# lambdaclass/ethrex

Measured on NVIDIA H100. Metric: bn254_g1_msm_points_per_sec, higher is better.
Workload: dtype u32x8 Montgomery (254-bit modular integer)

## Files before the change

ethrex_b200/csrc/msm.cu:

```cuda
#include "common.cuh"
#include "tma.cuh"
#include <cstdlib>

namespace b200zk {

static constexpr int kMaxWindows = 64;
static constexpr uint32_t kMaxPipelineChunks = 64;
static constexpr int kChunk = 16;
static constexpr int kG2MinBlocks = 1;

struct MsmPlan {
  uint32_t c, W, B;
  uint32_t chunk, T;
  uint32_t merged;
  uint32_t Wr;
  uint32_t table_stride;
  uint32_t adaptive;
};

uint32_t precompute_window(size_t n) {
  uint32_t lg = 0;
  while (((size_t)1 << lg) < n) ++lg;
  if (lg >= 20) return 20;
  if (lg <= 6) return 6;
// ... 134 lines not shown
#pragma unroll
    for (int u = 0; u < kScatterIlp; ++u) {
      const size_t t = t0 + u * stride;
      live[u] = t < total_pad;
      code[u] = (live[u] && t < total) ? __ldg(digits + t) : kNoDigit;
      active[u] = code[u] != kNoDigit;
      w[u] = live[u] ? t / n : 0;
      g[u] = (pl.merged ? 0u : (uint32_t)(w[u] * pl.B)) + (code[u] & 0x7fffffffu);
    }
#pragma unroll
    for (int u = 0; u < kScatterIlp; ++u) {
      base[u] = 0; rank[u] = 0; mask[u] = 0;
      if (live[u]) {
        uint32_t cnt = warp_group(g[u], active[u], &rank[u], &mask[u], pl.adaptive != 0);
        if (active[u] && rank[u] == 0) base[u] = atomicAdd(&cursor[g[u]], cnt);
      }
    }
#pragma unroll
    for (int u = 0; u < kScatterIlp; ++u) {
      if (live[u]) {
        uint32_t bs = __shfl_sync(mask[u], base[u], __ffs(mask[u]) - 1);
        const size_t t = t0 + u * stride;
        if (active[u]) idx[bs + rank[u]] = (uint32_t)((t - w[u] * n) + (pl.merged ? w[u] * pl.table_stride : 0)) | (code[u] & 0x80000000u);
      }
    }
  }
}

static constexpr uint32_t kSortTile = 1024;
static constexpr uint32_t kSortMaxW = 16;
static constexpr uint32_t kSortMaxBins = 1024;
static constexpr uint32_t kSortMaxFine = 2048;
static constexpr uint32_t kSortCountSub = 4;
static constexpr int kFineIlp = 8;

struct SortPlan {
  uint32_t fb;
  uint32_t C;
  uint32_t NC;
  uint32_t range;
  uint32_t G;
};
static bool make_sort_plan(size_t n, const MsmPlan& pl, int sm_count, SortPlan* sp) {
  const size_t G = (size_t)pl.Wr * pl.B;
  uint32_t kb = 0;
  while (((size_t)1 << kb) < G) ++kb;
  if (pl.W > kSortMaxW || kb < 12 || n < ((size_t)1 << 16)) return false;
  uint32_t cb = kb > 19 ? 10 : 9;
  if (kb - cb > 11) return false;
  sp->fb = kb - cb;
  sp->C = (uint32_t)((G + ((size_t)1 << sp->fb) - 1) >> sp->fb);
  sp->G = (uint32_t)G;
  uint32_t nc = (uint32_t)sm_count;
  size_t tiles = (n + kSortTile - 1) / kSortTile;
  if (nc > tiles) nc = (uint32_t)tiles;
  size_t per = ((tiles + nc - 1) / nc) * kSortTile;
  sp->NC = (uint32_t)((n + per - 1) / per);
  sp->range = (uint32_t)per;
  return true;
}

B2_D void recode_scalar(const uint32_t s[8], const MsmPlan& pl, uint32_t (&code)[kSortMaxW]) {
  uint32_t carry = 0;
#pragma unroll
  for (uint32_t w = 0; w < kSortMaxW; ++w) {
    code[w] = kNoDigit;
    if (w < pl.W) {
      uint32_t coef = window_bits(s, w, pl.c) + carry;
      carry = 0;
      uint32_t neg = 0, mag = coef;
      if (w + 1 < pl.W && coef >= pl.B) { carry = 1; neg = 0x80000000u; mag = (1u << pl.c) - coef; }
      code[w] = mag ? ((mag - 1) | neg) : kNoDigit;
    }
  }
}

__global__ void __launch_bounds__(kHistTile) msm_sort_count(const void* scalars, size_t n, uint32_t flags, MsmPlan pl, SortPlan sp, uint32_t* cnt) {
  __shared__ __align__(128) uint4 tile[2][kHistTile * 2];
  __shared__ uint64_t bar[2];
  __shared__ uint32_t sh[kSortMaxBins];
  const uint32_t r = blockIdx.x / kSortCountSub, sub = blockIdx.x % kSortCountSub;
  for (uint32_t b = threadIdx.x; b < sp.C; b += kHistTile) sh[b] = 0;
  const size_t lo = (size_t)r * sp.range, hi = lo + sp.range < n ? lo + sp.range : n;
  const size_t tiles_all = lo < hi ? (hi - lo + kHistTile - 1) / kHistTile : 0;
  const size_t per = (tiles_all + kSortCountSub - 1) / kSortCountSub;
  const size_t t0 = sub * per, t1 = t0 + per < tiles_all ? t0 + per : tiles_all;
  if (threadIdx.x == 0) { tma::barrier_init(&bar[0], 1); tma::barrier_init(&bar[1], 1); tma::barrier_init_fence(); }
  __syncthreads();
  auto issue = [&](size_t tl, uint32_t buf) {
    size_t first = lo + tl * kHistTile;
    uint32_t bytes = (uint32_t)((hi - first < kHistTile ? hi - first : kHistTile) * 32);
    tma::barrier_expect(&bar[buf], bytes);
    tma::bulk_load(tile[buf], reinterpret_cast<const uint8_t*>(scalars) + first * 32, bytes, &bar[buf]);
  };
  if (threadIdx.x == 0 && t0 < t1) issue(t0, 0);
  uint32_t it = 0;
  for (size_t tl = t0; tl < t1; ++tl, ++it) {
    const uint32_t buf = it & 1;
    if (threadIdx.x == 0 && tl + 1 < t1) issue(tl + 1, buf ^ 1);
    tma::barrier_wait(&bar[buf], (it >> 1) & 1);
    const size_t i = lo + tl * kHistTile + threadIdx.x;
    if (i < hi) {
      uint32_t s[8], code[kSortMaxW];
      decode_scalar(tile[buf][2 * threadIdx.x], tile[buf][2 * threadIdx.x + 1], flags, s);
      recode_scalar(s, pl, code);
#pragma unroll
      for (uint32_t w = 0; w < kSortMaxW; ++w)
        if (code[w] != kNoDigit) {
          const uint32_t g = (pl.merged ? 0u : w * pl.B) + (code[w] & 0x7fffffffu);
          atomicAdd(&sh[g >> sp.fb], 1u);
        }
    }
    __syncthreads();
  }
  __syncthreads();
  for (uint32_t b = threadIdx.x; b < sp.C; b += kHistTile) if (sh[b]) atomicAdd(&cnt[(size_t)b * sp.NC + r], sh[b]);
}

struct SortCoarseSmem {
  uint2 ent[kSortTile * kSortMaxW];
  uint32_t dst[kSortTile * kSortMaxW];
  uint32_t run_base[kSortMaxBins], tile_cnt[kSortMaxBins], tile_start[kSortMaxBins];
  uint32_t warp_tot[kSortTile / 32];
  uint32_t total;
};
__global__ void __launch_bounds__(kSortTile, 1) msm_sort_coarse(const void* __restrict__ scalars, size_t n, uint32_t flags, MsmPlan pl, SortPlan sp, const uint32_t* __restrict__ base,
                                                               uint2* __restrict__ ent1) {
  extern __shared__ __align__(16) uint8_t smem_raw[];
  SortCoarseSmem& sm = *reinterpret_cast<SortCoarseSmem*>(smem_raw);
  const uint32_t r = blockIdx.x, tid = threadIdx.x;
  const size_t lo = (size_t)r * sp.range, hi = lo + sp.range < n ? lo + sp.range : n;
  const uint32_t fmask = (1u << sp.fb) - 1u;
  for (uint32_t b = tid; b < sp.C; b += kSortTile) { sm.run_base[b] = __ldg(base + (size_t)b * sp.NC + r); sm.tile_cnt[b] = 0; }
  __syncthreads();
  const uint4* sc = reinterpret_cast<const uint4*>(scalars);
  for (size_t t0 = lo; t0 < hi; t0 += kSortTile) {
    const size_t i = t0 + tid;
    uint32_t code[kSortMaxW], rank[kSortMaxW];
    const bool live = i < hi;
#pragma unroll
    for (uint32_t w = 0; w < kSortMaxW; ++w) { code[w] = kNoDigit; rank[w] = 0; }
    if (live) {
      uint32_t s[8];
      decode_scalar(__ldg(sc + 2 * i), __ldg(sc + 2 * i + 1), flags, s);
      recode_scalar(s, pl, code);
#pragma unroll
      for (uint32_t w = 0; w < kSortMaxW; ++w)
        if (code[w] != kNoDigit) {
          const uint32_t g = (pl.merged ? 0u : w * pl.B) + (code[w] & 0x7fffffffu);
          rank[w] = atomicAdd(&sm.tile_cnt[g >> sp.fb], 1u);
        }
    }
    __syncthreads();
    {
      const uint32_t v = tid < sp.C ? sm.tile_cnt[tid] : 0;
      uint32_t incl = v;
#pragma unroll
      for (int o = 1; o < 32; o <<= 1) { uint32_t t = __shfl_up_sync(0xffffffffu, incl, o); if ((tid & 31) >= (unsigned)o) incl += t; }
      if ((tid & 31) == 31) sm.warp_tot[tid >> 5] = incl;
      __syncthreads();
      uint32_t wb = 0;
      for (uint32_t k = 0; k < (tid >> 5); ++k) wb += sm.warp_tot[k];
      if (tid < sp.C) sm.tile_start[tid] = wb + incl - v;
      if (tid == kSortTile - 1) sm.total = wb + incl;
    }
    __syncthreads();
    if (live) {
#pragma unroll
      for (uint32_t w = 0; w < kSortMaxW; ++w)
        if (code[w] != kNoDigit) {
          const uint32_t g = (pl.merged ? 0u : w * pl.B) + (code[w] & 0x7fffffffu);
          const uint32_t b = g >> sp.fb, pos = sm.tile_start[b] + rank[w];
          sm.ent[pos] = make_uint2((uint32_t)(i + (pl.merged ? (size_t)w * pl.table_stride : 0)) | (code[w] & 0x80000000u), g & fmask);
          sm.dst[pos] = sm.run_base[b] + rank[w];
        }
    }
    __syncthreads();
    const uint32_t total = sm.total;
    for (uint32_t t = tid; t < total; t += kSortTile) ent1[sm.dst[t]] = sm.ent[t];
    __syncthreads();
    if (tid < sp.C) { sm.run_base[tid] += sm.tile_cnt[tid]; sm.tile_cnt[tid] = 0; }
    __syncthreads();
  }
}

static constexpr uint32_t kFineTile = 8192;
static constexpr uint32_t kFineSeg = 4 * kFineTile;
struct SortFineSmem {
  uint32_t val[kFineTile], dst[kFineTile];
  uint32_t cur[kSortMaxFine], tcnt[kSortMaxFine], tstart[kSortMaxFine];
  uint32_t warp_tot[32];
  uint32_t total;
};
B2_D void scan_fine_keys(const uint32_t* in, uint32_t* out, uint32_t F, uint32_t* warp_tot, uint32_t* total) {
  const uint32_t tid = threadIdx.x, k0 = 2 * tid, k1 = 2 * tid + 1;
  const uint32_t v0 = k0 < F ? in[k0] : 0, v1 = k1 < F ? in[k1] : 0;
  uint32_t incl = v0 + v1;
#pragma unroll
  for (int o = 1; o < 32; o <<= 1) { uint32_t t = __shfl_up_sync(0xffffffffu, incl, o); if ((tid & 31) >= (unsigned)o) incl += t; }
  if ((tid & 31) == 31) warp_tot[tid >> 5] = incl;
  __syncthreads();
  uint32_t wb = 0;
  for (uint32_t k = 0; k < (tid >> 5); ++k) wb += warp_tot[k];
  const uint32_t ex = wb + incl - v0 - v1;
  if (k0 < F) out[k0] = ex;
  if (k1 < F) out[k1] = ex + v0;
  if (tid == 1023) *total = wb + incl;
  __syncthreads();
}
__global__ void __launch_bounds__(1024) msm_sort_items(const uint32_t* __restrict__ base, SortPlan sp, uint32_t* __restrict__ item_start) {
  __shared__ uint32_t wt[32];
  const uint32_t tid = threadIdx.x;
  uint32_t v = 0;
  if (tid < sp.C) { const uint32_t sz = __ldg(base + (size_t)(tid + 1) * sp.NC) - __ldg(base + (size_t)tid * sp.NC); v = (sz + kFineSeg - 1) / kFineSeg; }
  uint32_t incl = v;
#pragma unroll
  for (int o = 1; o < 32; o <<= 1) { uint32_t t = __shfl_up_sync(0xffffffffu, incl, o); if ((tid & 31) >= (unsigned)o) incl += t; }
  if ((tid & 31) == 31) wt[tid >> 5] = incl;
  __syncthreads();
  uint32_t wb = 0;
  for (uint32_t k = 0; k < (tid >> 5); ++k) wb += wt[k];
  if (tid < sp.C) item_start[tid] = wb + incl - v;
  if (tid == sp.C - 1) item_start[sp.C] = wb + incl;
}
B2_D uint32_t item_bin(const uint32_t* __restrict__ item_start, uint32_t C, uint32_t i) {
  uint32_t lo = 0, hi = C;
  while (hi - lo > 1) { uint32_t mid = (lo + hi) >> 1; if (__ldg(item_start + mid) <= i) lo = mid; else hi = mid; }
  return lo;
}
__global__ void __launch_bounds__(1024, 2) msm_sort_fine_count(const uint2* __restrict__ ent1, SortPlan sp, const uint32_t* __restrict__ base, const uint32_t* __restrict__ item_start,
                                                               uint32_t* __restrict__ cnt2) {
  __shared__ uint32_t fh[kSortMaxFine];
  const uint32_t i = blockIdx.x, tid = threadIdx.x, F = 1u << sp.fb;
  if (i >= __ldg(item_start + sp.C)) return;
  const uint32_t b = item_bin(item_start, sp.C, i);
  const uint32_t bs = __ldg(base + (size_t)b * sp.NC), be = __ldg(base + (size_t)(b + 1) * sp.NC);
  const uint32_t s0 = bs + (i - __ldg(item_start + b)) * kFineSeg, s1 = (be - s0 > kFineSeg) ? s0 + kFineSeg : be;
  for (uint32_t k = tid; k < F; k += 1024) fh[k] = 0;
  __syncthreads();
  for (uint32_t e0 = s0 + tid; e0 < s1; e0 += 1024 * kFineIlp) {
    uint32_t kk[kFineIlp];
#pragma unroll
    for (int u = 0; u < kFineIlp; ++u) { const uint32_t e = e0 + u * 1024; kk[u] = e < s1 ? __ldg(&ent1[e].y) : 0xffffffffu; }
#pragma unroll
    for (int u = 0; u < kFineIlp; ++u) if (kk[u] != 0xffffffffu) atomicAdd(&fh[kk[u]], 1u);
  }
  __syncthreads();
  for (uint32_t k = tid; k < F; k += 1024) cnt2[(size_t)i * F + k] = fh[k];
}
__global__ void __launch_bounds__(256) msm_sort_fine_prefix(SortPlan sp, const uint32_t* __restrict__ item_start, uint32_t* __restrict__ cnt2, uint32_t* __restrict__ hist) {
  const uint32_t F = 1u << sp.fb;
  const size_t t = blockIdx.x * (size_t)blockDim.x + threadIdx.x;
  if (t >= (size_t)sp.C * F) return;
  const uint32_t b = (uint32_t)(t >> sp.fb), k = (uint32_t)t & (F - 1);
  const uint32_t i0 = __ldg(item_start + b), i1 = __ldg(item_start + b + 1);
  uint32_t run = 0;
  for (uint32_t i = i0; i < i1; ++i) {
    const size_t at = (size_t)i * F + k;
    const uint32_t c = cnt2[at];
    cnt2[at] = run;
    run += c;
  }
  if (t < sp.G) hist[t] = run;
}
__global__ void __launch_bounds__(1024, 1) msm_sort_fine_place(const uint2* __restrict__ ent1, SortPlan sp, const uint32_t* __restrict__ base, const uint32_t* __restrict__ item_start,
                                                               const uint32_t* __restrict__ cnt2, const uint32_t* __restrict__ offsets, uint32_t* __restrict__ idx) {
  extern __shared__ __align__(16) uint8_t smem_raw[];
  SortFineSmem& sm = *reinterpret_cast<SortFineSmem*>(smem_raw);
  const uint32_t i = blockIdx.x, tid = threadIdx.x, F = 1u << sp.fb;
  if (i >= __ldg(item_start + sp.C)) return;
  const uint32_t b = item_bin(item_start, sp.C, i);
  const uint32_t bs = __ldg(base + (size_t)b * sp.NC), be = __ldg(base + (size_t)(b + 1) * sp.NC);
  const uint32_t s0 = bs + (i - __ldg(item_start + b)) * kFineSeg, s1 = (be - s0 > kFineSeg) ? s0 + kFineSeg : be;
  for (uint32_t k = tid; k < F; k += 1024) {
    const size_t g = (size_t)b * F + k;
    sm.cur[k] = (g < sp.G ? __ldg(offsets + g) : 0u) + __ldg(cnt2 + (size_t)i * F + k);
    sm.tcnt[k] = 0;
  }
  __syncthreads();
  for (uint32_t t0 = s0; t0 < s1; t0 += kFineTile) {
    uint2 ev[kFineTile / 1024];
    uint32_t rank[kFineTile / 1024];
#pragma unroll
    for (int u = 0; u < (int)(kFineTile / 1024); ++u) {
      const uint32_t e = t0 + u * 1024 + tid;
      ev[u] = e < s1 ? __ldg(ent1 + e) : make_uint2(0u, 0xffffffffu);
    }
#pragma unroll
    for (int u = 0; u < (int)(kFineTile / 1024); ++u) rank[u] = ev[u].y != 0xffffffffu ? atomicAdd(&sm.tcnt[ev[u].y], 1u) : 0u;
    __syncthreads();
    scan_fine_keys(sm.tcnt, sm.tstart, F, sm.warp_tot, &sm.total);
#pragma unroll
    for (int u = 0; u < (int)(kFineTile / 1024); ++u)
      if (ev[u].y != 0xffffffffu) {
        const uint32_t pos = sm.tstart[ev[u].y] + rank[u];
        sm.val[pos] = ev[u].x;
        sm.dst[pos] = sm.cur[ev[u].y] + rank[u];
      }
    __syncthreads();
    const uint32_t total = sm.total;
    for (uint32_t t = tid; t < total; t += 1024) idx[sm.dst[t]] = sm.val[t];
    __syncthreads();
    for (uint32_t k = tid; k < F; k += 1024) { sm.cur[k] += sm.tcnt[k]; sm.tcnt[k] = 0; }
    __syncthreads();
  }
}

static constexpr int kScanThreads = 256, kScanItems = 8, kScanTile = kScanThreads * kScanItems;

B2_D uint32_t scan_value(const uint32_t* in, const uint32_t* aux, size_t i, uint32_t seg, uint32_t shift) {
  uint32_t v = in[i];
  if (!seg) return (v + (1u << shift) - 1u) >> shift;
  return (v != 0 && (aux[i] % seg) != 0) ? 1u : 0u;
}

__global__ void __launch_bounds__(kScanThreads) scan_tile_sums(const uint32_t* in, const uint32_t* aux, size_t G, uint32_t seg, uint32_t shift, uint32_t* tile_sums) {
  __shared__ uint32_t red[kScanThreads / 32];
  size_t base = (size_t)blockIdx.x * kScanTile + (size_t)threadIdx.x * kScanItems;
  uint32_t s = 0;
#pragma unroll
  for (int k = 0; k < kScanItems; ++k) if (base + k < G) s += scan_value(in, aux, base + k, seg, shift);
#pragma unroll
  for (int o = 16; o; o >>= 1) s += __shfl_xor_sync(0xffffffffu, s, o);
  if ((threadIdx.x & 31) == 0) red[threadIdx.x >> 5] = s;
  __syncthreads();
  if (threadIdx.x == 0) {
    uint32_t t = 0;
    for (int k = 0; k < kScanThreads / 32; ++k) t += red[k];
    tile_sums[blockIdx.x] = t;
  }
// ... 684 lines not shown
  B2_LAUNCH(ctx, groth16_assemble_zk, 3, 32, 0, st, (const uint8_t*)d_partials, count, d_g1_terms, d_g2_terms, zk, (uint8_t*)d_out);
  return B200ZK_OK;
}

static inline void phase_mark(b200zk_ctx* ctx, int k, cudaStream_t st) {
  if (ctx->profiling) cudaEventRecord(ctx->ev[k], st);
}

static int g2_pair_knob() {
  static int k = -1;
  if (k < 0) { const char* e = getenv("B200ZK_G2_PAIR"); k = (e && (*e == '0' || *e == '3' || *e == '4')) ? (*e - '0') : 3; }
  return k;
}
template <class F> static size_t resident_slices(const b200zk_ctx* ctx) {
  if (IsFq2<F>::value) { const int k = g2_pair_knob(); return (size_t)ctx->sm_count * (k ? 64u * (unsigned)k : 256u); }
  return (size_t)ctx->sm_count * (sizeof(F) > 32 ? 256u : 512u);
}
template <class F>
static int launch_accumulate(b200zk_ctx* ctx, cudaStream_t st, const void* pts, const uint32_t* idx, const uint32_t* offsets, const uint32_t* run_off, uint32_t G, uint32_t L,
                             size_t slices, void* partials, uint32_t* run_bucket) {
  const unsigned agrid = (unsigned)((slices + 127) / 128);
  if constexpr (IsFq2<F>::value) {
    const int k = g2_pair_knob();
    const unsigned pgrid = (unsigned)((2 * slices + 127) / 128);
    if (k == 3) B2_LAUNCH(ctx, msm_accumulate_g2_pair<3>, pgrid, 128, 0, st, pts, idx, offsets, run_off, G, L, partials, run_bucket);
    else if (k == 4) B2_LAUNCH(ctx, msm_accumulate_g2_pair<4>, pgrid, 128, 0, st, pts, idx, offsets, run_off, G, L, partials, run_bucket);
    else B2_LAUNCH(ctx, (msm_accumulate<F, false, 1>), agrid, 128, 0, st, pts, idx, offsets, run_off, G, L, partials, run_bucket);
  } else {
    B2_LAUNCH(ctx, (msm_accumulate<F, false>), agrid, 128, 0, st, pts, idx, offsets, run_off, G, L, partials, run_bucket);
  }
  return B200ZK_OK;
}

static int legacy_sort_knob() {
  static int knob = -1;
  if (knob < 0) { const char* e = getenv("B200ZK_SORT"); knob = (e && !strcmp(e, "legacy")) ? 1 : 0; }
  return knob;
}
static double chunk_ratio_knob(double dflt) {
  const char* e = getenv("B200ZK_CHUNK_RATIO");
  double r = (e && *e) ? atof(e) : dflt;
  return (r >= 1.0 && r <= 64.0) ? r : dflt;
}
static size_t sort_ctab_bytes(int sm_count) { return (2 * ((size_t)kSortMaxBins * (size_t)sm_count + 1) + kSortMaxBins + 1) * 4; }
static size_t sort_cnt2_bytes(size_t M_max) { return (M_max / kFineSeg + kSortMaxBins + 1) * (size_t)kSortMaxFine * 4; }
static int run_two_level_sort(b200zk_ctx* ctx, const void* d_scalars, size_t n, uint32_t flags, const MsmPlan& pl, const SortPlan& sp, uint32_t* hist, uint32_t* offsets,
                              uint32_t* tsum, uint2* ent1, uint32_t* ctab, uint32_t* cnt2, uint32_t* idx, cudaStream_t st, bool mark) {
  const size_t Gc = (size_t)sp.C * sp.NC, tilesC = (Gc + kScanTile - 1) / kScanTile;
  const size_t G = sp.G, tilesG = (G + kScanTile - 1) / kScanTile;
  uint32_t *cnt = ctab, *base = ctab + Gc + 1, *item_start = base + Gc + 1;
  if (!ctx->attr_sort) {
    B2_CUDA(ctx, cudaFuncSetAttribute(msm_sort_coarse, cudaFuncAttributeMaxDynamicSharedMemorySize, (int)sizeof(SortCoarseSmem)));
    B2_CUDA(ctx, cudaFuncSetAttribute(msm_sort_fine_place, cudaFuncAttributeMaxDynamicSharedMemorySize, (int)sizeof(SortFineSmem)));
    ctx->attr_sort = true;
  }
  B2_CUDA(ctx, cudaMemsetAsync(cnt, 0, (Gc + 1) * 4, st));
  B2_LAUNCH(ctx, msm_sort_count, sp.NC * kSortCountSub, kHistTile, 0, st, d_scalars, n, flags, pl, sp, cnt);
  if (mark) phase_mark(ctx, 1, st);
  B2_LAUNCH(ctx, scan_tile_sums, (unsigned)tilesC, kScanThreads, 0, st, (const uint32_t*)cnt, (const uint32_t*)nullptr, Gc, 0u, 0u, tsum);
  B2_LAUNCH(ctx, scan_tile_offsets, 1, 1024, 0, st, tsum, tilesC);
  B2_LAUNCH(ctx, scan_apply, (unsigned)tilesC, kScanThreads, 0, st, (const uint32_t*)cnt, (const uint32_t*)nullptr, Gc, 0u, 0u, (const uint32_t*)tsum, base, (uint32_t*)nullptr);
  if (mark) phase_mark(ctx, 2, st);
  B2_LAUNCH(ctx, msm_sort_coarse, sp.NC, kSortTile, sizeof(SortCoarseSmem), st, d_scalars, n, flags, pl, sp, (const uint32_t*)base, ent1);
  const unsigned max_items = (unsigned)((n * (size_t)pl.W) / kFineSeg + sp.C + 1);
  const uint32_t F = 1u << sp.fb;
  B2_LAUNCH(ctx, msm_sort_items, 1, 1024, 0, st, (const uint32_t*)base, sp, item_start);
  B2_LAUNCH(ctx, msm_sort_fine_count, max_items, 1024, 0, st, (const uint2*)ent1, sp, (const uint32_t*)base, (const uint32_t*)item_start, cnt2);
  B2_LAUNCH(ctx, msm_sort_fine_prefix, (unsigned)(((size_t)sp.C * F + 255) / 256), 256, 0, st, sp, (const uint32_t*)item_start, cnt2, hist);
  B2_LAUNCH(ctx, scan_tile_sums, (unsigned)tilesG, kScanThreads, 0, st, (const uint32_t*)hist, (const uint32_t*)nullptr, G, 0u, 0u, tsum);
  B2_LAUNCH(ctx, scan_tile_offsets, 1, 1024, 0, st, tsum, tilesG);
  B2_LAUNCH(ctx, scan_apply, (unsigned)tilesG, kScanThreads, 0, st, (const uint32_t*)hist, (const uint32_t*)nullptr, G, 0u, 0u, (const uint32_t*)tsum, offsets, (uint32_t*)nullptr);
  B2_LAUNCH(ctx, msm_sort_fine_place, max_items, 1024, sizeof(SortFineSmem), st, (const uint2*)ent1, sp, (const uint32_t*)base, (const uint32_t*)item_start, (const uint32_t*)cnt2,
            (const uint32_t*)offsets, idx);
  return B200ZK_OK;
}

template <class F>
static int msm_run_pipelined(b200zk_ctx* ctx, const void* d_points, const void* d_scalars, const void* h_scalars, size_t n, uint32_t flags,
                             cudaStream_t st, void* d_partial, const MsmPlan& pl, uint32_t K) {
  const size_t G = (size_t)pl.Wr * pl.B;
  const size_t tiles = (G + kScanTile - 1) / kScanTile;
  const size_t xy = 4 * FieldBytes<F>::value, pt = 2 * FieldBytes<F>::value;
  size_t bnd[kMaxPipelineChunks + 1];
  uint32_t chunks = 0;
  {
    const double r = h_scalars ? chunk_ratio_knob(IsFq2<F>::value ? 12.0 : 4.0) : 1.0;
    double tot = 0, w = 1;
    for (uint32_t k = 0; k < K; ++k) { tot += w; w *= r; }
    double cum = 0; w = 1;
    bnd[0] = 0;
    for (uint32_t k = 0; k < K; ++k) {
      cum += w; w *= r;
      size_t hi = (k == K - 1) ? n : std::min(n, (((size_t)((double)n * (cum / tot))) + 1023) & ~(size_t)1023);
      if (hi > bnd[chunks]) bnd[++chunks] = hi;
    }
  }
  size_t chunk = 0;
  for (uint32_t k = 0; k < chunks; ++k) chunk = std::max(chunk, bnd[k + 1] - bnd[k]);
  const size_t Mk_max = chunk * pl.W;
  const size_t resident = resident_slices<F>(ctx);
  uint32_t Lk[kMaxPipelineChunks];
  size_t S_max = 0;
  for (uint32_t k = 0; k < chunks; ++k) {
    const size_t Mk = (bnd[k + 1] - bnd[k]) * pl.W;
    Lk[k] = pick_slice_len(Mk, resident);
    S_max = std::max(S_max, Mk / Lk[k] + 1 + G);
  }
  SortPlan sp0;
  const bool two_level = !legacy_sort_knob() && make_sort_plan(chunk, pl, ctx->sm_count, &sp0);
  const size_t Gc = (size_t)kSortMaxBins * (size_t)ctx->sm_count;
  for (int sl = 0; sl < 2; ++sl) {
    SortSlot& s = ctx->slot[sl];
    B2_TRY(ensure(ctx, s.hist, G * 4)); B2_TRY(ensure(ctx, s.offsets, (G + 1) * 4)); B2_TRY(ensure(ctx, s.cursor, G * 4));
    B2_TRY(ensure(ctx, s.run_off, (G + 1) * 4));
    B2_TRY(ensure(ctx, s.tsum, std::max(tiles, (Gc + kScanTile - 1) / kScanTile) * 4));
    B2_TRY(ensure(ctx, s.digits, Mk_max * 4)); B2_TRY(ensure(ctx, s.idx, Mk_max * 4));
    if (two_level) { B2_TRY(ensure(ctx, s.key, Mk_max * 8)); B2_TRY(ensure(ctx, s.ctab, sort_ctab_bytes(ctx->sm_count))); B2_TRY(ensure(ctx, s.cnt2, sort_cnt2_bytes(Mk_max))); }
  }
  B2_TRY(ensure(ctx, ctx->ws_buckets, S_max * xy));
  B2_TRY(ensure(ctx, ctx->ws_segbucket, S_max * 4));
  B2_TRY(ensure(ctx, ctx->ws_totals, G * xy));
  B2_TRY(ensure(ctx, ctx->ws_chunkS, (size_t)pl.Wr * pl.T * xy));
  B2_TRY(ensure(ctx, ctx->ws_chunkV, (size_t)pl.Wr * pl.T * xy));
  if (h_scalars) B2_TRY(ensure(ctx, ctx->ws_scalars, n * 32 + 32));
  const uint8_t* dsc = (const uint8_t*)(h_scalars ? ctx->ws_scalars.p : d_scalars);
  cudaStream_t cs = ctx->stream_sort;
  if (h_scalars) {
    B2_CUDA(ctx, cudaEventRecord(ctx->ev_in, st));
    B2_CUDA(ctx, cudaStreamWaitEvent(cs, ctx->ev_in, 0));
    if (chunks > kMaxPipelineChunks) return fail(ctx, B200ZK_ERR_INVALID_ARG, "msm: too many pipeline chunks");
    for (uint32_t k = 0; k < chunks; ++k) {
      const size_t lo = bnd[k], nk = bnd[k + 1] - lo;
      B2_CUDA(ctx, cudaMemcpyAsync((void*)(dsc + lo * 32), (const uint8_t*)h_scalars + lo * 32, nk * 32, cudaMemcpyHostToDevice, cs));
      B2_CUDA(ctx, cudaEventRecord(ctx->ev_up[k], cs));
    }
  }
  auto sort_chunk = [&](uint32_t k) -> int {
    const size_t lo = bnd[k], nk = bnd[k + 1] - lo;
    const uint32_t L = Lk[k];
    SortSlot& s = ctx->slot[k & 1];
    uint32_t *hist = (uint32_t*)s.hist.p, *offsets = (uint32_t*)s.offsets.p, *cursor = (uint32_t*)s.cursor.p, *run_off = (uint32_t*)s.run_off.p,
             *tsum = (uint32_t*)s.tsum.p, *digits = (uint32_t*)s.digits.p, *idx = (uint32_t*)s.idx.p;
    if (h_scalars) B2_CUDA(ctx, cudaStreamWaitEvent(st, ctx->ev_up[k], 0));
    SortPlan sp;
    const bool tl = two_level && make_sort_plan(nk, pl, ctx->sm_count, &sp);
    if (tl) {
      B2_TRY(run_two_level_sort(ctx, (const void*)(dsc + lo * 32), nk, flags, pl, sp, hist, offsets, tsum, (uint2*)s.key.p, (uint32_t*)s.ctab.p, (uint32_t*)s.cnt2.p, idx, st, false));
    } else {
      B2_CUDA(ctx, cudaMemsetAsync(hist, 0, G * 4, st));
      const unsigned sgrid = (unsigned)std::min<size_t>((nk + 255) / 256, (size_t)ctx->sm_count * 8);
      B2_LAUNCH(ctx, msm_hist, sgrid, 256, 0, st, (const void*)(dsc + lo * 32), nk, flags, pl, hist, digits);
      B2_LAUNCH(ctx, scan_tile_sums, (unsigned)tiles, kScanThreads, 0, st, hist, (const uint32_t*)nullptr, G, 0u, 0u, tsum);
      B2_LAUNCH(ctx, scan_tile_offsets, 1, 1024, 0, st, tsum, tiles);
      B2_LAUNCH(ctx, scan_apply, (unsigned)tiles, kScanThreads, 0, st, hist, (const uint32_t*)nullptr, G, 0u, 0u, tsum, offsets, cursor);
      const unsigned wgrid = (unsigned)std::min<size_t>((nk * (size_t)pl.W + 255) / 256, (size_t)ctx->sm_count * 32);
      B2_LAUNCH(ctx, msm_scatter, wgrid, 256, 0, st, (const uint32_t*)digits, nk, pl, cursor, idx);
    }
    B2_LAUNCH(ctx, scan_tile_sums, (unsigned)tiles, kScanThreads, 0, st, hist, (const uint32_t*)offsets, G, L, 0u, tsum);
    B2_LAUNCH(ctx, scan_tile_offsets, 1, 1024, 0, st, tsum, tiles);
    B2_LAUNCH(ctx, scan_apply, (unsigned)tiles, kScanThreads, 0, st, hist, (const uint32_t*)offsets, G, L, 0u, tsum, run_off, (uint32_t*)nullptr);
    return B200ZK_OK;
  };
  for (uint32_t k = 0; k < chunks; ++k) {
    const size_t lo = bnd[k], nk = bnd[k + 1] - lo;
    const uint32_t L = Lk[k];
    const size_t slices = (nk * pl.W + L - 1) / L;
    B2_TRY(sort_chunk(k));
    SortSlot& s = ctx->slot[k & 1];
    const void* pts = (const uint8_t*)d_points + lo * pt;
    B2_TRY(launch_accumulate<F>(ctx, st, pts, (const uint32_t*)s.idx.p, (const uint32_t*)s.offsets.p, (const uint32_t*)s.run_off.p, (uint32_t)G, L, slices, ctx->ws_buckets.p,
                                (uint32_t*)ctx->ws_segbucket.p));
    {
      size_t worst_entries = (pl.merged ? nk * (size_t)pl.W : nk) + 1;
      size_t worst = (worst_entries + L - 1) / L + 1;
      for (size_t stride = 1; stride < worst; stride *= kTreeRadix)
        B2_LAUNCH(ctx, partial_tree<F>, (unsigned)((S_max + 127) / 128), 128, 0, st, (const uint32_t*)s.run_off.p, (const uint32_t*)ctx->ws_segbucket.p, (uint32_t)G, (uint32_t)stride, ctx->ws_buckets.p);
    }
    B2_LAUNCH(ctx, bucket_merge<F>, (unsigned)((G + 127) / 128), 128, 0, st, (const void*)ctx->ws_buckets.p, (const uint32_t*)s.run_off.p, (uint32_t)G, k == 0 ? 1 : 0, ctx->ws_totals.p);
  }
  const size_t nchunks = (size_t)pl.Wr * pl.T;
// ... 58 lines not shown
  B2_TRY(ensure(ctx, ctx->ws_blocksums, tiles * 4));
  B2_TRY(ensure(ctx, ctx->ws_idx, n * (size_t)pl.W * 4));
  B2_TRY(ensure(ctx, ctx->ws_digits, n * (size_t)pl.W * 4));
  const size_t M_max = n * (size_t)pl.W;
  uint32_t rounds = 0;
  if (ctx->msm_pair_rounds >= 0) rounds = (uint32_t)ctx->msm_pair_rounds;
  if (rounds > 4) rounds = 4;
  if (rounds && M_max >= ((size_t)1 << 31)) rounds = 0;
  if (sort_mode) rounds = 0;
  const uint32_t kSegLen = pick_slice_len(M_max >> rounds, resident_slices<F>(ctx));
  const size_t S_max = (M_max >> rounds) / kSegLen + 1 + G;
  const size_t slices = ((M_max >> rounds) + G + kSegLen - 1) / kSegLen;
  if (rounds) {
    const size_t pt = 2 * FieldBytes<F>::value;
    B2_TRY(ensure(ctx, ctx->ws_q1, (M_max / 2 + G + 1) * pt));
    if (rounds > 1) B2_TRY(ensure(ctx, ctx->ws_q0, (M_max / 4 + G + 1) * pt));
    B2_TRY(ensure(ctx, ctx->ws_prefix, (M_max / 2 + G + 1) * FieldBytes<F>::value));
    B2_TRY(ensure(ctx, ctx->ws_info, (M_max / 2 + G + 1) * 4));
    B2_TRY(ensure(ctx, ctx->ws_pairoff0, (G + 1) * 4));
    B2_TRY(ensure(ctx, ctx->ws_pairoff1, (G + 1) * 4));
  }
  B2_TRY(ensure(ctx, ctx->ws_buckets, S_max * xy));
  B2_TRY(ensure(ctx, ctx->ws_segoff, (G + 1) * 4));
  B2_TRY(ensure(ctx, ctx->ws_segbucket, S_max * 4));
  B2_TRY(ensure(ctx, ctx->ws_chunkS, (size_t)pl.Wr * pl.T * xy));
  B2_TRY(ensure(ctx, ctx->ws_chunkV, (size_t)pl.Wr * pl.T * xy));
  uint32_t* hist = (uint32_t*)ctx->ws_hist.p;
  uint32_t* offsets = (uint32_t*)ctx->ws_offsets.p;
  uint32_t* cursor = (uint32_t*)ctx->ws_cursor.p;
  uint32_t* tsum = (uint32_t*)ctx->ws_blocksums.p;
  uint32_t* idx = (uint32_t*)ctx->ws_idx.p;

  SortPlan sp;
  const bool two_level = !legacy_sort_knob() && make_sort_plan(n, pl, ctx->sm_count, &sp);
  if (two_level) {
    B2_TRY(ensure(ctx, ctx->ws_key, M_max * 8));
    B2_TRY(ensure(ctx, ctx->ws_ctab, sort_ctab_bytes(ctx->sm_count)));
    B2_TRY(ensure(ctx, ctx->ws_cnt2, sort_cnt2_bytes(M_max)));
    B2_TRY(ensure(ctx, ctx->ws_blocksums, (std::max(tiles, ((size_t)sp.C * sp.NC + kScanTile - 1) / kScanTile)) * 4));
    tsum = (uint32_t*)ctx->ws_blocksums.p;
  }
  phase_mark(ctx, 0, st);
  nvtxRangePushA("b200zk:msm_sort");
  if (sort_mode != 2 && two_level) {
    B2_TRY(run_two_level_sort(ctx, d_scalars, n, flags, pl, sp, hist, offsets, tsum, (uint2*)ctx->ws_key.p, (uint32_t*)ctx->ws_ctab.p, (uint32_t*)ctx->ws_cnt2.p, idx, st, true));
  } else if (sort_mode != 2) {
    B2_CUDA(ctx, cudaMemsetAsync(hist, 0, G * 4, st));
    const unsigned sgrid = (unsigned)std::min<size_t>((n + 255) / 256, (size_t)ctx->sm_count * 8);
    uint32_t* digits = (uint32_t*)ctx->ws_digits.p;
    B2_LAUNCH(ctx, msm_hist, sgrid, 256, 0, st, d_scalars, n, flags, pl, hist, digits);
    phase_mark(ctx, 1, st);
    B2_LAUNCH(ctx, scan_tile_sums, (unsigned)tiles, kScanThreads, 0, st, hist, (const uint32_t*)nullptr, G, 0u, 0u, tsum);
    B2_LAUNCH(ctx, scan_tile_offsets, 1, 1024, 0, st, tsum, tiles);
    B2_LAUNCH(ctx, scan_apply, (unsigned)tiles, kScanThreads, 0, st, hist, (const uint32_t*)nullptr, G, 0u, 0u, tsum, offsets, cursor);
    phase_mark(ctx, 2, st);
    const unsigned wgrid = (unsigned)std::min<size_t>((n * (size_t)pl.W + 255) / 256, (size_t)ctx->sm_count * 32);
    B2_LAUNCH(ctx, msm_scatter, wgrid, 256, 0, st, (const uint32_t*)digits, n, pl, cursor, idx);
  } else {
    phase_mark(ctx, 1, st);
    phase_mark(ctx, 2, st);
  }
  nvtxRangePop();
  phase_mark(ctx, 3, st);
  NvtxRange nvtx_acc("b200zk:msm_accumulate+reduce");
  const uint32_t* cur_off = offsets;
  const void* cur_pts = d_points;
  for (uint32_t r = 1; r <= rounds; ++r) {
    uint32_t* off_r = (uint32_t*)(r & 1 ? ctx->ws_pairoff1.p : ctx->ws_pairoff0.p);
    B2_LAUNCH(ctx, scan_tile_sums, (unsigned)tiles, kScanThreads, 0, st, hist, (const uint32_t*)nullptr, G, 0u, r, tsum);
    B2_LAUNCH(ctx, scan_tile_offsets, 1, 1024, 0, st, tsum, tiles);
    B2_LAUNCH(ctx, scan_apply, (unsigned)tiles, kScanThreads, 0, st, hist, (const uint32_t*)nullptr, G, 0u, r, tsum, off_r, (uint32_t*)nullptr);
    const size_t out_max = (M_max >> r) + G;
    void* q = (r & 1) ? ctx->ws_q1.p : ctx->ws_q0.p;
    const unsigned pgrid = (unsigned)((out_max / kPairBatch + 1 + 127) / 128);
    if (r == 1) B2_LAUNCH(ctx, (pair_sum<F, true>), pgrid, 128, 0, st, cur_pts, (const uint32_t*)idx, cur_off, (const uint32_t*)off_r, (uint32_t)G, ctx->ws_prefix.p, (uint32_t*)ctx->ws_info.p, q);
    else B2_LAUNCH(ctx, (pair_sum<F, false>), pgrid, 128, 0, st, cur_pts, (const uint32_t*)idx, cur_off, (const uint32_t*)off_r, (uint32_t)G, ctx->ws_prefix.p, (uint32_t*)ctx->ws_info.p, q);
    cur_off = off_r;
    cur_pts = q;
// ... 88 lines not shown
```

Before: 403.3 million.

## Pack two-level sort intermediate entries into 32 bits and prefetch fine tiles

The coarse sort pass now writes 4-byte packed entries holding the run-local index, window, sign bit and fine key, instead of 8-byte uint2 entries, whenever the bit budget fits. The fine place pass rebuilds the global point index by binary-searching the coarse run boundaries, which are kept in shared memory. It also adds L2 prefetches for the next tile. The aim is to halve the global traffic of the intermediate key buffer, at the cost of extra integer work and binary searches in the fine pass. A 'wide' environment knob keeps the old layout.

```diff
diff --git a/ethrex_b200/csrc/msm.cu b/ethrex_b200/csrc/msm.cu
--- a/ethrex_b200/csrc/msm.cu
+++ b/ethrex_b200/csrc/msm.cu
@@ -190,6 +190,7 @@
 static constexpr uint32_t kSortMaxBins = 1024;
 static constexpr uint32_t kSortMaxFine = 2048;
 static constexpr uint32_t kSortCountSub = 4;
+static constexpr uint32_t kSortMaxNC = 256;
 static constexpr int kFineIlp = 8;
 
 struct SortPlan {
@@ -198,8 +199,10 @@
   uint32_t NC;
   uint32_t range;
   uint32_t G;
+  uint32_t packed;
+  uint32_t wb;
 };
-static bool make_sort_plan(size_t n, const MsmPlan& pl, int sm_count, SortPlan* sp) {
+static bool make_sort_plan(size_t n, const MsmPlan& pl, int sm_count, bool wide, SortPlan* sp) {
   const size_t G = (size_t)pl.Wr * pl.B;
   uint32_t kb = 0;
   while (((size_t)1 << kb) < G) ++kb;
@@ -209,14 +212,25 @@
   sp->fb = kb - cb;
   sp->C = (uint32_t)((G + ((size_t)1 << sp->fb) - 1) >> sp->fb);
   sp->G = (uint32_t)G;
-  uint32_t nc = (uint32_t)sm_count;
+  uint32_t nc = sm_count < (int)kSortMaxNC ? (uint32_t)sm_count : kSortMaxNC;
   size_t tiles = (n + kSortTile - 1) / kSortTile;
   if (nc > tiles) nc = (uint32_t)tiles;
   size_t per = ((tiles + nc - 1) / nc) * kSortTile;
   sp->NC = (uint32_t)((n + per - 1) / per);
   sp->range = (uint32_t)per;
+  uint32_t rb = 0, wb = 0;
+  while ((1u << rb) < sp->range) ++rb;
+  while ((1u << wb) < pl.W) ++wb;
+  sp->wb = wb;
+  sp->packed = (!wide && rb + wb + 1 + sp->fb <= 32) ? 1u : 0u;
   return true;
 }
+
+B2_D uint32_t pack_entry(const SortPlan& sp, uint32_t local, uint32_t w, uint32_t code, uint32_t key) {
+  return (local << (sp.fb + 1 + sp.wb)) | (w << (sp.fb + 1)) | ((code >> 31) << sp.fb) | key;
+}
+B2_D uint32_t fine_key(uint32_t e, uint32_t fmask) { return e & fmask; }
+B2_D uint32_t fine_key(uint2 e, uint32_t) { return e.y; }
 
 B2_D void recode_scalar(const uint32_t s[8], const MsmPlan& pl, uint32_t (&code)[kSortMaxW]) {
   uint32_t carry = 0;
@@ -275,17 +289,19 @@
   for (uint32_t b = threadIdx.x; b < sp.C; b += kHistTile) if (sh[b]) atomicAdd(&cnt[(size_t)b * sp.NC + r], sh[b]);
 }
 
+template <class E>
 struct SortCoarseSmem {
-  uint2 ent[kSortTile * kSortMaxW];
+  E ent[kSortTile * kSortMaxW];
   uint32_t dst[kSortTile * kSortMaxW];
   uint32_t run_base[kSortMaxBins], tile_cnt[kSortMaxBins], tile_start[kSortMaxBins];
   uint32_t warp_tot[kSortTile / 32];
   uint32_t total;
 };
+template <class E>
 __global__ void __launch_bounds__(kSortTile, 1) msm_sort_coarse(const void* __restrict__ scalars, size_t n, uint32_t flags, MsmPlan pl, SortPlan sp, const uint32_t* __restrict__ base,
-                                                               uint2* __restrict__ ent1) {
+                                                               E* __restrict__ ent1) {
   extern __shared__ __align__(16) uint8_t smem_raw[];
-  SortCoarseSmem& sm = *reinterpret_cast<SortCoarseSmem*>(smem_raw);
+  SortCoarseSmem<E>& sm = *reinterpret_cast<SortCoarseSmem<E>*>(smem_raw);
   const uint32_t r = blockIdx.x, tid = threadIdx.x;
   const size_t lo = (size_t)r * sp.range, hi = lo + sp.range < n ? lo + sp.range : n;
   const uint32_t fmask = (1u << sp.fb) - 1u;
@@ -329,7 +345,11 @@
         if (code[w] != kNoDigit) {
           const uint32_t g = (pl.merged ? 0u : w * pl.B) + (code[w] & 0x7fffffffu);
           const uint32_t b = g >> sp.fb, pos = sm.tile_start[b] + rank[w];
-          sm.ent[pos] = make_uint2((uint32_t)(i + (pl.merged ? (size_t)w * pl.table_stride : 0)) | (code[w] & 0x80000000u), g & fmask);
+          if constexpr (sizeof(E) == 4) {
+            sm.ent[pos] = pack_entry(sp, (uint32_t)(i - lo), w, code[w], g & fmask);
+          } else {
+            sm.ent[pos] = make_uint2((uint32_t)(i + (pl.merged ? (size_t)w * pl.table_stride : 0)) | (code[w] & 0x80000000u), g & fmask);
+          }
           sm.dst[pos] = sm.run_base[b] + rank[w];
         }
     }
@@ -347,9 +367,14 @@
 struct SortFineSmem {
   uint32_t val[kFineTile], dst[kFineTile];
   uint32_t cur[kSortMaxFine], tcnt[kSortMaxFine], tstart[kSortMaxFine];
+  uint32_t run[kSortMaxNC + 1];
   uint32_t warp_tot[32];
   uint32_t total;
 };
+B2_D uint32_t run_of(const uint32_t* run, uint32_t lo, uint32_t hi, uint32_t e) {
+  while (hi - lo > 1) { const uint32_t mid = (lo + hi) >> 1; if (run[mid] <= e) lo = mid; else hi = mid; }
+  return lo;
+}
 B2_D void scan_fine_keys(const uint32_t* in, uint32_t* out, uint32_t F, uint32_t* warp_tot, uint32_t* total) {
   const uint32_t tid = threadIdx.x, k0 = 2 * tid, k1 = 2 * tid + 1;
   const uint32_t v0 = k0 < F ? in[k0] : 0, v1 = k1 < F ? in[k1] : 0;
@@ -386,7 +411,8 @@
   while (hi - lo > 1) { uint32_t mid = (lo + hi) >> 1; if (__ldg(item_start + mid) <= i) lo = mid; else hi = mid; }
   return lo;
 }
-__global__ void __launch_bounds__(1024, 2) msm_sort_fine_count(const uint2* __restrict__ ent1, SortPlan sp, const uint32_t* __restrict__ base, const uint32_t* __restrict__ item_start,
+template <class E>
+__global__ void __launch_bounds__(1024, 2) msm_sort_fine_count(const E* __restrict__ ent1, SortPlan sp, const uint32_t* __restrict__ base, const uint32_t* __restrict__ item_start,
                                                                uint32_t* __restrict__ cnt2) {
   __shared__ uint32_t fh[kSortMaxFine];
   const uint32_t i = blockIdx.x, tid = threadIdx.x, F = 1u << sp.fb;
@@ -399,7 +425,11 @@
   for (uint32_t e0 = s0 + tid; e0 < s1; e0 += 1024 * kFineIlp) {
     uint32_t kk[kFineIlp];
 #pragma unroll
-    for (int u = 0; u < kFineIlp; ++u) { const uint32_t e = e0 + u * 1024; kk[u] = e < s1 ? __ldg(&ent1[e].y) : 0xffffffffu; }
+    for (int u = 0; u < kFineIlp; ++u) {
+      const uint32_t e = e0 + u * 1024;
+      if constexpr (sizeof(E) == 4) kk[u] = e < s1 ? fine_key(__ldg(ent1 + e), F - 1) : 0xffffffffu;
+      else kk[u] = e < s1 ? __ldg(&ent1[e].y) : 0xffffffffu;
+    }
 #pragma unroll
     for (int u = 0; u < kFineIlp; ++u) if (kk[u] != 0xffffffffu) atomicAdd(&fh[kk[u]], 1u);
   }
@@ -421,8 +451,11 @@
   }
   if (t < sp.G) hist[t] = run;
 }
-__global__ void __launch_bounds__(1024, 1) msm_sort_fine_place(const uint2* __restrict__ ent1, SortPlan sp, const uint32_t* __restrict__ base, const uint32_t* __restrict__ item_start,
+template <class E>
+__global__ void __launch_bounds__(1024, 1) msm_sort_fine_place(const E* __restrict__ ent1, MsmPlan pl, SortPlan sp, const uint32_t* __restrict__ base, const uint32_t* __restrict__ item_start,
                                                                const uint32_t* __restrict__ cnt2, const uint32_t* __restrict__ offsets, uint32_t* __restrict__ idx) {
+  constexpr bool kPacked = sizeof(E) == 4;
+  constexpr int kPer = (int)(kFineTile / 1024);
   extern __shared__ __align__(16) uint8_t smem_raw[];
   SortFineSmem& sm = *reinterpret_cast<SortFineSmem*>(smem_raw);
   const uint32_t i = blockIdx.x, tid = threadIdx.x, F = 1u << sp.fb;
@@ -430,30 +463,53 @@
   const uint32_t b = item_bin(item_start, sp.C, i);
   const uint32_t bs = __ldg(base + (size_t)b * sp.NC), be = __ldg(base + (size_t)(b + 1) * sp.NC);
   const uint32_t s0 = bs + (i - __ldg(item_start + b)) * kFineSeg, s1 = (be - s0 > kFineSeg) ? s0 + kFineSeg : be;
+  auto prefetch_tile = [&](uint32_t t) {
+    const uint32_t bytes = t < s1 ? (s1 - t < kFineTile ? s1 - t : kFineTile) * (uint32_t)sizeof(E) : 0u;
+    for (uint32_t l = tid * 128; l < bytes; l += 1024 * 128) asm volatile("prefetch.global.L2 [%0];" ::"l"(reinterpret_cast<const uint8_t*>(ent1 + t) + l));
+  };
+  prefetch_tile(s0);
   for (uint32_t k = tid; k < F; k += 1024) {
     const size_t g = (size_t)b * F + k;
     sm.cur[k] = (g < sp.G ? __ldg(offsets + g) : 0u) + __ldg(cnt2 + (size_t)i * F + k);
     sm.tcnt[k] = 0;
   }
+  if constexpr (kPacked)
+    for (uint32_t r = tid; r <= sp.NC; r += 1024) sm.run[r] = __ldg(base + (size_t)b * sp.NC + r);
   __syncthreads();
+  const uint32_t lshift = sp.fb + 1 + sp.wb, wmask = (1u << sp.wb) - 1u;
   for (uint32_t t0 = s0; t0 < s1; t0 += kFineTile) {
-    uint2 ev[kFineTile / 1024];
-    uint32_t rank[kFineTile / 1024];
-#pragma unroll
-    for (int u = 0; u < (int)(kFineTile / 1024); ++u) {
+    prefetch_tile(t0 + kFineTile);
+    E ev[kPer];
+    uint32_t key[kPer], rank[kPer];
+#pragma unroll
+    for (int u = 0; u < kPer; ++u) {
       const uint32_t e = t0 + u * 1024 + tid;
-      ev[u] = e < s1 ? __ldg(ent1 + e) : make_uint2(0u, 0xffffffffu);
-    }
-#pragma unroll
-    for (int u = 0; u < (int)(kFineTile / 1024); ++u) rank[u] = ev[u].y != 0xffffffffu ? atomicAdd(&sm.tcnt[ev[u].y], 1u) : 0u;
+      if (e < s1) { ev[u] = __ldg(ent1 + e); key[u] = fine_key(ev[u], F - 1); }
+      else { ev[u] = E{}; key[u] = 0xffffffffu; }
+    }
+#pragma unroll
+    for (int u = 0; u < kPer; ++u) rank[u] = key[u] != 0xffffffffu ? atomicAdd(&sm.tcnt[key[u]], 1u) : 0u;
     __syncthreads();
     scan_fine_keys(sm.tcnt, sm.tstart, F, sm.warp_tot, &sm.total);
-#pragma unroll
-    for (int u = 0; u < (int)(kFineTile / 1024); ++u)
-      if (ev[u].y != 0xffffffffu) {
-        const uint32_t pos = sm.tstart[ev[u].y] + rank[u];
-        sm.val[pos] = ev[u].x;
-        sm.dst[pos] = sm.cur[ev[u].y] + rank[u];
+    uint32_t r_lo = 0, r_hi = 0;
+    if constexpr (kPacked) {
+      r_lo = run_of(sm.run, 0, sp.NC, t0);
+      r_hi = run_of(sm.run, r_lo, sp.NC, (s1 - t0 > kFineTile ? t0 + kFineTile : s1) - 1) + 1;
+    }
+#pragma unroll
+    for (int u = 0; u < kPer; ++u)
+      if (key[u] != 0xffffffffu) {
+        const uint32_t pos = sm.tstart[key[u]] + rank[u];
+        uint32_t v;
+        if constexpr (kPacked) {
+          const uint32_t e = ev[u], r = run_of(sm.run, r_lo, r_hi, t0 + u * 1024 + tid);
+          const uint32_t w = (e >> (sp.fb + 1)) & wmask;
+          v = (r * sp.range + (e >> lshift) + (pl.merged ? w * pl.table_stride : 0u)) | (((e >> sp.fb) & 1u) << 31);
+        } else {
+          v = ev[u].x;
+        }
+        sm.val[pos] = v;
+        sm.dst[pos] = sm.cur[key[u]] + rank[u];
       }
     __syncthreads();
     const uint32_t total = sm.total;
@@ -1204,11 +1260,14 @@
   return B200ZK_OK;
 }
 
-static int legacy_sort_knob() {
-  static int knob = -1;
-  if (knob < 0) { const char* e = getenv("B200ZK_SORT"); knob = (e && !strcmp(e, "legacy")) ? 1 : 0; }
-  return knob;
-}
+enum SortKnob { kSortAuto = 0, kSortLegacy = 1, kSortWide = 2 };
+static SortKnob sort_knob() {
+  const char* e = getenv("B200ZK_SORT");
+  if (e && !strcmp(e, "legacy")) return kSortLegacy;
+  if (e && !strcmp(e, "wide")) return kSortWide;
+  return kSortAuto;
+}
+static size_t sort_entry_bytes(const SortPlan& sp) { return sp.packed ? 4 : 8; }
 static double chunk_ratio_knob(double dflt) {
   const char* e = getenv("B200ZK_CHUNK_RATIO");
   double r = (e && *e) ? atof(e) : dflt;
@@ -1216,14 +1275,17 @@
 }
 static size_t sort_ctab_bytes(int sm_count) { return (2 * ((size_t)kSortMaxBins * (size_t)sm_count + 1) + kSortMaxBins + 1) * 4; }
 static size_t sort_cnt2_bytes(size_t M_max) { return (M_max / kFineSeg + kSortMaxBins + 1) * (size_t)kSortMaxFine * 4; }
-static int run_two_level_sort(b200zk_ctx* ctx, const void* d_scalars, size_t n, uint32_t flags, const MsmPlan& pl, const SortPlan& sp, uint32_t* hist, uint32_t* offsets,
-                              uint32_t* tsum, uint2* ent1, uint32_t* ctab, uint32_t* cnt2, uint32_t* idx, cudaStream_t st, bool mark) {
+template <class E>
+static int run_two_level_sort_e(b200zk_ctx* ctx, const void* d_scalars, size_t n, uint32_t flags, const MsmPlan& pl, const SortPlan& sp, uint32_t* hist, uint32_t* offsets,
+                              uint32_t* tsum, E* ent1, uint32_t* ctab, uint32_t* cnt2, uint32_t* idx, cudaStream_t st, bool mark) {
   const size_t Gc = (size_t)sp.C * sp.NC, tilesC = (Gc + kScanTile - 1) / kScanTile;
   const size_t G = sp.G, tilesG = (G + kScanTile - 1) / kScanTile;
   uint32_t *cnt = ctab, *base = ctab + Gc + 1, *item_start = base + Gc + 1;
   if (!ctx->attr_sort) {
-    B2_CUDA(ctx, cudaFuncSetAttribute(msm_sort_coarse, cudaFuncAttributeMaxDynamicSharedMemorySize, (int)sizeof(SortCoarseSmem)));
-    B2_CUDA(ctx, cudaFuncSetAttribute(msm_sort_fine_place, cudaFuncAttributeMaxDynamicSharedMemorySize, (int)sizeof(SortFineSmem)));
+    B2_CUDA(ctx, cudaFuncSetAttribute(msm_sort_coarse<uint32_t>, cudaFuncAttributeMaxDynamicSharedMemorySize, (int)sizeof(SortCoarseSmem<uint32_t>)));
+    B2_CUDA(ctx, cudaFuncSetAttribute(msm_sort_coarse<uint2>, cudaFuncAttributeMaxDynamicSharedMemorySize, (int)sizeof(SortCoarseSmem<uint2>)));
+    B2_CUDA(ctx, cudaFuncSetAttribute(msm_sort_fine_place<uint32_t>, cudaFuncAttributeMaxDynamicSharedMemorySize, (int)sizeof(SortFineSmem)));
+    B2_CUDA(ctx, cudaFuncSetAttribute(msm_sort_fine_place<uint2>, cudaFuncAttributeMaxDynamicSharedMemorySize, (int)sizeof(SortFineSmem)));
     ctx->attr_sort = true;
   }
   B2_CUDA(ctx, cudaMemsetAsync(cnt, 0, (Gc + 1) * 4, st));
@@ -1233,18 +1295,23 @@
   B2_LAUNCH(ctx, scan_tile_offsets, 1, 1024, 0, st, tsum, tilesC);
   B2_LAUNCH(ctx, scan_apply, (unsigned)tilesC, kScanThreads, 0, st, (const uint32_t*)cnt, (const uint32_t*)nullptr, Gc, 0u, 0u, (const uint32_t*)tsum, base, (uint32_t*)nullptr);
   if (mark) phase_mark(ctx, 2, st);
-  B2_LAUNCH(ctx, msm_sort_coarse, sp.NC, kSortTile, sizeof(SortCoarseSmem), st, d_scalars, n, flags, pl, sp, (const uint32_t*)base, ent1);
+  B2_LAUNCH(ctx, msm_sort_coarse<E>, sp.NC, kSortTile, sizeof(SortCoarseSmem<E>), st, d_scalars, n, flags, pl, sp, (const uint32_t*)base, ent1);
   const unsigned max_items = (unsigned)((n * (size_t)pl.W) / kFineSeg + sp.C + 1);
   const uint32_t F = 1u << sp.fb;
   B2_LAUNCH(ctx, msm_sort_items, 1, 1024, 0, st, (const uint32_t*)base, sp, item_start);
-  B2_LAUNCH(ctx, msm_sort_fine_count, max_items, 1024, 0, st, (const uint2*)ent1, sp, (const uint32_t*)base, (const uint32_t*)item_start, cnt2);
+  B2_LAUNCH(ctx, msm_sort_fine_count<E>, max_items, 1024, 0, st, (const E*)ent1, sp, (const uint32_t*)base, (const uint32_t*)item_start, cnt2);
   B2_LAUNCH(ctx, msm_sort_fine_prefix, (unsigned)(((size_t)sp.C * F + 255) / 256), 256, 0, st, sp, (const uint32_t*)item_start, cnt2, hist);
   B2_LAUNCH(ctx, scan_tile_sums, (unsigned)tilesG, kScanThreads, 0, st, (const uint32_t*)hist, (const uint32_t*)nullptr, G, 0u, 0u, tsum);
   B2_LAUNCH(ctx, scan_tile_offsets, 1, 1024, 0, st, tsum, tilesG);
   B2_LAUNCH(ctx, scan_apply, (unsigned)tilesG, kScanThreads, 0, st, (const uint32_t*)hist, (const uint32_t*)nullptr, G, 0u, 0u, (const uint32_t*)tsum, offsets, (uint32_t*)nullptr);
-  B2_LAUNCH(ctx, msm_sort_fine_place, max_items, 1024, sizeof(SortFineSmem), st, (const uint2*)ent1, sp, (const uint32_t*)base, (const uint32_t*)item_start, (const uint32_t*)cnt2,
+  B2_LAUNCH(ctx, msm_sort_fine_place<E>, max_items, 1024, sizeof(SortFineSmem), st, (const E*)ent1, pl, sp, (const uint32_t*)base, (const uint32_t*)item_start, (const uint32_t*)cnt2,
             (const uint32_t*)offsets, idx);
   return B200ZK_OK;
+}
+static int run_two_level_sort(b200zk_ctx* ctx, const void* d_scalars, size_t n, uint32_t flags, const MsmPlan& pl, const SortPlan& sp, uint32_t* hist, uint32_t* offsets,
+                              uint32_t* tsum, void* ent1, uint32_t* ctab, uint32_t* cnt2, uint32_t* idx, cudaStream_t st, bool mark) {
+  if (sp.packed) return run_two_level_sort_e(ctx, d_scalars, n, flags, pl, sp, hist, offsets, tsum, (uint32_t*)ent1, ctab, cnt2, idx, st, mark);
+  return run_two_level_sort_e(ctx, d_scalars, n, flags, pl, sp, hist, offsets, tsum, (uint2*)ent1, ctab, cnt2, idx, st, mark);
 }
 
 template <class F>
@@ -1279,7 +1346,8 @@
     S_max = std::max(S_max, Mk / Lk[k] + 1 + G);
   }
   SortPlan sp0;
-  const bool two_level = !legacy_sort_knob() && make_sort_plan(chunk, pl, ctx->sm_count, &sp0);
+  const SortKnob knob = sort_knob();
+  const bool two_level = knob != kSortLegacy && make_sort_plan(chunk, pl, ctx->sm_count, knob == kSortWide, &sp0);
   const size_t Gc = (size_t)kSortMaxBins * (size_t)ctx->sm_count;
   for (int sl = 0; sl < 2; ++sl) {
     SortSlot& s = ctx->slot[sl];
@@ -1287,7 +1355,7 @@
     B2_TRY(ensure(ctx, s.run_off, (G + 1) * 4));
     B2_TRY(ensure(ctx, s.tsum, std::max(tiles, (Gc + kScanTile - 1) / kScanTile) * 4));
     B2_TRY(ensure(ctx, s.digits, Mk_max * 4)); B2_TRY(ensure(ctx, s.idx, Mk_max * 4));
-    if (two_level) { B2_TRY(ensure(ctx, s.key, Mk_max * 8)); B2_TRY(ensure(ctx, s.ctab, sort_ctab_bytes(ctx->sm_count))); B2_TRY(ensure(ctx, s.cnt2, sort_cnt2_bytes(Mk_max))); }
+    if (two_level) { B2_TRY(ensure(ctx, s.key, Mk_max * sort_entry_bytes(sp0))); B2_TRY(ensure(ctx, s.ctab, sort_ctab_bytes(ctx->sm_count))); B2_TRY(ensure(ctx, s.cnt2, sort_cnt2_bytes(Mk_max))); }
   }
   B2_TRY(ensure(ctx, ctx->ws_buckets, S_max * xy));
   B2_TRY(ensure(ctx, ctx->ws_segbucket, S_max * 4));
@@ -1315,9 +1383,9 @@
              *tsum = (uint32_t*)s.tsum.p, *digits = (uint32_t*)s.digits.p, *idx = (uint32_t*)s.idx.p;
     if (h_scalars) B2_CUDA(ctx, cudaStreamWaitEvent(st, ctx->ev_up[k], 0));
     SortPlan sp;
-    const bool tl = two_level && make_sort_plan(nk, pl, ctx->sm_count, &sp);
+    const bool tl = two_level && make_sort_plan(nk, pl, ctx->sm_count, knob == kSortWide, &sp);
     if (tl) {
-      B2_TRY(run_two_level_sort(ctx, (const void*)(dsc + lo * 32), nk, flags, pl, sp, hist, offsets, tsum, (uint2*)s.key.p, (uint32_t*)s.ctab.p, (uint32_t*)s.cnt2.p, idx, st, false));
+      B2_TRY(run_two_level_sort(ctx, (const void*)(dsc + lo * 32), nk, flags, pl, sp, hist, offsets, tsum, s.key.p, (uint32_t*)s.ctab.p, (uint32_t*)s.cnt2.p, idx, st, false));
     } else {
       B2_CUDA(ctx, cudaMemsetAsync(hist, 0, G * 4, st));
       const unsigned sgrid = (unsigned)std::min<size_t>((nk + 255) / 256, (size_t)ctx->sm_count * 8);
@@ -1442,9 +1510,10 @@
   uint32_t* idx = (uint32_t*)ctx->ws_idx.p;
 
   SortPlan sp;
-  const bool two_level = !legacy_sort_knob() && make_sort_plan(n, pl, ctx->sm_count, &sp);
+  const SortKnob knob = sort_knob();
+  const bool two_level = knob != kSortLegacy && make_sort_plan(n, pl, ctx->sm_count, knob == kSortWide, &sp);
   if (two_level) {
-    B2_TRY(ensure(ctx, ctx->ws_key, M_max * 8));
+    B2_TRY(ensure(ctx, ctx->ws_key, M_max * sort_entry_bytes(sp)));
     B2_TRY(ensure(ctx, ctx->ws_ctab, sort_ctab_bytes(ctx->sm_count)));
     B2_TRY(ensure(ctx, ctx->ws_cnt2, sort_cnt2_bytes(M_max)));
     B2_TRY(ensure(ctx, ctx->ws_blocksums, (std::max(tiles, ((size_t)sp.C * sp.NC + kScanTile - 1) / kScanTile)) * 4));
@@ -1453,7 +1522,7 @@
   phase_mark(ctx, 0, st);
   nvtxRangePushA("b200zk:msm_sort");
   if (sort_mode != 2 && two_level) {
-    B2_TRY(run_two_level_sort(ctx, d_scalars, n, flags, pl, sp, hist, offsets, tsum, (uint2*)ctx->ws_key.p, (uint32_t*)ctx->ws_ctab.p, (uint32_t*)ctx->ws_cnt2.p, idx, st, true));
+    B2_TRY(run_two_level_sort(ctx, d_scalars, n, flags, pl, sp, hist, offsets, tsum, ctx->ws_key.p, (uint32_t*)ctx->ws_ctab.p, (uint32_t*)ctx->ws_cnt2.p, idx, st, true));
   } else if (sort_mode != 2) {
     B2_CUDA(ctx, cudaMemsetAsync(hist, 0, G * 4, st));
     const unsigned sgrid = (unsigned)std::min<size_t>((n + 255) / 256, (size_t)ctx->sm_count * 8);
```

Result: faster. 409.3 million, median of 6 (+1.5%).
